# facebookresearch/moolib

Measured on AMD Instinct MI355X. Metric: env frames/sec (whole node) IMPALA Atari-ResNet, higher is better.
Workload: dtype bf16; 1 GPU; model=IMPALA Atari deep ResNet (16/32/32ch, FC3872-256), global_batch=32, seq_len=20, parallelism=dp1, actor_batch_size=128, num_actor_batches=2, num_actor_cpus=10, virtual_batch_size=32, num_actions=18, frame=84x84x4 uint8

## Files before the change

### hip/conv3x3.hip.inc

```

namespace conv3x3 {

using bf16 = __bf16;
using bf16x8 = __attribute__((ext_vector_type(8))) __bf16;
using floatx4 = __attribute__((ext_vector_type(4))) float;

#define C3_DEV static __device__ __forceinline__

C3_DEV bf16x8 zero8() {
  bf16x8 z;
#pragma unroll
  for (int e = 0; e < 8; ++e) z[e] = (bf16)0.f;
  return z;
}

enum { kEpiNone = 0, kEpiBias = 1, kEpiBiasRelu = 2, kEpiBiasAdd = 3 };

template <int C, bool RELU_IN, int RT>
__global__ __launch_bounds__(256) void conv3x3_nhwc_kernel(
    const bf16* __restrict__ x,
    const bf16* __restrict__ wPacked,
    const bf16* __restrict__ biasIn,
    bf16* __restrict__ out,
    const bf16* __restrict__ bias1,
    const bf16* __restrict__ res,
    const bf16* __restrict__ bias2,
    int NB, int H, int W, int K, int epi) {
  constexpr int KK = (9 * C + 31) / 32;
  const int lane = threadIdx.x & 63;
  const int wave = threadIdx.x >> 6;
  const int lo = lane & 15, hi = lane >> 4;
  const int64_t M = (int64_t)NB * H * W;
  const int64_t pixBase = ((int64_t)blockIdx.x * 4 + wave) * (16 * RT);
  if (pixBase >= M) return;

  int an[RT], aoh[RT], aow[RT];
  bool aok[RT];
#pragma unroll
  for (int rt = 0; rt < RT; ++rt) {
    const int64_t apix = pixBase + rt * 16 + lo;
    aok[rt] = apix < M;
    an[rt] = aoh[rt] = aow[rt] = 0;
    if (aok[rt]) {
      int64_t r = apix;
      aow[rt] = (int)(r % W);
      r /= W;
      aoh[rt] = (int)(r % H);
      an[rt] = (int)(r / H);
    }
  }
  const int nCt = K >> 4;
  constexpr int CH = (RT == 1) ? 2 : RT;
  floatx4 acc[CH][2];
#pragma unroll
  for (int ch = 0; ch < CH; ++ch)
#pragma unroll
    for (int ct = 0; ct < 2; ++ct) acc[ch][ct] = (floatx4){0.f, 0.f, 0.f, 0.f};

#pragma unroll
  for (int kk = 0; kk < KK; ++kk) {
    const int kd = kk * 32 + hi * 8;
    const int tap = kd / C;
    const int c0 = kd % C;
    bf16x8 a[RT];
#pragma unroll
    for (int rt = 0; rt < RT; ++rt) {
      a[rt] = zero8();
      if (aok[rt] && tap < 9) {
        const int ih = aoh[rt] + tap / 3 - 1;
        const int iw = aow[rt] + tap % 3 - 1;
        if (ih >= 0 && ih < H && iw >= 0 && iw < W) {
          const bf16* p = x + ((((int64_t)an[rt] * H + ih) * W + iw) * C + c0);
          a[rt] = *reinterpret_cast<const bf16x8*>(p);
          if (RELU_IN) {
#pragma unroll
            for (int e = 0; e < 8; ++e) {
              float v = (float)a[rt][e];
              if (biasIn != nullptr) v += (float)biasIn[c0 + e];
              a[rt][e] = (bf16)(v > 0.f ? v : 0.f);
            }
          }
        }
      }
    }
    for (int ct = 0; ct < nCt; ++ct) {
      const bf16* bp = wPacked + (((int64_t)ct * KK + kk) * 64 + lane) * 8;
      bf16x8 b = *reinterpret_cast<const bf16x8*>(bp);
#pragma unroll
      for (int rt = 0; rt < RT; ++rt) {
        const int ch = (RT == 1) ? (kk & 1) : rt;
        acc[ch][ct] = __builtin_amdgcn_mfma_f32_16x16x32_bf16(a[rt], b, acc[ch][ct], 0, 0, 0);
      }
    }
  }

#pragma unroll
  for (int rt = 0; rt < RT; ++rt) {
    for (int ct = 0; ct < nCt; ++ct) {
      const int col = ct * 16 + lo;
      const float b1 = (bias1 != nullptr) ? (float)bias1[col] : 0.f;
      const float b2 = (bias2 != nullptr) ? (float)bias2[col] : 0.f;
#pragma unroll
      for (int reg = 0; reg < 4; ++reg) {
        const int64_t pix = pixBase + rt * 16 + hi * 4 + reg;
        if (pix >= M) continue;
        float v = (RT == 1) ? (acc[0][ct][reg] + acc[1][ct][reg]) : acc[rt][ct][reg];
        if (epi == kEpiBias) {
          v += b1;
        } else if (epi == kEpiBiasRelu) {
          v += b1;
          v = v > 0.f ? v : 0.f;
        } else if (epi == kEpiBiasAdd) {
          v += b1 + b2 + (float)res[pix * K + col];
        }
        out[pix * K + col] = (bf16)v;
      }
    }
  }
}

template <int C, bool RELU_IN>
__global__ __launch_bounds__(256) void conv3x3_nhwc_lds_kernel(
    const bf16* __restrict__ x, const bf16* __restrict__ wPacked,
    const bf16* __restrict__ biasIn, bf16* __restrict__ out,
    const bf16* __restrict__ bias1, const bf16* __restrict__ res,
    const bf16* __restrict__ bias2, int NB, int H, int W, int K, int epi, int BR) {
  constexpr int KK = (9 * C + 31) / 32;
  const int lane = threadIdx.x & 63;
  const int wave = threadIdx.x >> 6;
  const int lo = lane & 15, hi = lane >> 4;
  const int nCt = K >> 4;
  const int WS = W + 2;

  extern __shared__ char smem[];
  bf16* slab = reinterpret_cast<bf16*>(smem);

  const int bandsPerImage = (H + BR - 1) / BR;
  const int band = blockIdx.x % bandsPerImage;
  const int n = blockIdx.x / bandsPerImage;
  const int row0 = band * BR;
  const int bandRows = min(BR, H - row0);
  const int bandPix = bandRows * W;

  constexpr int C8 = C / 8;
  {
    for (int idx = threadIdx.x; idx < (BR + 2) * WS * C8; idx += blockDim.x) {
      int c8 = idx % C8;
      int rest = idx / C8;
      int col = rest % WS;
      int sr = rest / WS;
      if (sr >= bandRows + 2) break;
      const int ih = row0 + sr - 1;
      const int iw = col - 1;
      bf16x8 v = zero8();
      if (ih >= 0 && ih < H && iw >= 0 && iw < W) {
        v = *reinterpret_cast<const bf16x8*>(
            x + ((((int64_t)n * H + ih) * W + iw) * C + c8 * 8));
        if (RELU_IN) {
#pragma unroll
          for (int e = 0; e < 8; ++e) {
            float f = (float)v[e];
            if (biasIn != nullptr) f += (float)biasIn[c8 * 8 + e];
            v[e] = (bf16)(f > 0.f ? f : 0.f);
          }
        }
      }
      *reinterpret_cast<bf16x8*>(slab + ((int64_t)sr * WS + col) * C + c8 * 8) = v;
    }
  }
  __syncthreads();

  const int nTiles = (bandPix + 15) / 16;
  for (int tile = wave; tile < nTiles; tile += 4) {
    const int p = tile * 16 + lo;
    const bool aok = p < bandPix;
    const int pr = aok ? p / W : 0;
    const int pc = aok ? p % W : 0;
    floatx4 acc[2][2];
#pragma unroll
    for (int pq = 0; pq < 2; ++pq)
#pragma unroll
      for (int ct = 0; ct < 2; ++ct) acc[pq][ct] = (floatx4){0.f, 0.f, 0.f, 0.f};
#pragma unroll
    for (int kk = 0; kk < KK; ++kk) {
      const int kd = kk * 32 + hi * 8;
      const int tap = kd / C;
      const int c0 = kd % C;
      bf16x8 a = zero8();
      if (aok && tap < 9) {
        const int sr = pr + tap / 3;
        const int sc = pc + tap % 3;
        a = *reinterpret_cast<const bf16x8*>(slab + ((int64_t)sr * WS + sc) * C + c0);
      }
      for (int ct = 0; ct < nCt; ++ct) {
        const bf16* bp = wPacked + (((int64_t)ct * KK + kk) * 64 + lane) * 8;
        bf16x8 b = *reinterpret_cast<const bf16x8*>(bp);
        acc[kk & 1][ct] = __builtin_amdgcn_mfma_f32_16x16x32_bf16(a, b, acc[kk & 1][ct], 0, 0, 0);
      }
    }
    const int64_t imgBase = ((int64_t)n * H + row0) * W;
    for (int ct = 0; ct < nCt; ++ct) {
      const int col = ct * 16 + lo;
      const float b1 = (bias1 != nullptr) ? (float)bias1[col] : 0.f;
      const float b2 = (bias2 != nullptr) ? (float)bias2[col] : 0.f;
#pragma unroll
      for (int reg = 0; reg < 4; ++reg) {
        const int pp = tile * 16 + hi * 4 + reg;
        if (pp >= bandPix) continue;
        const int64_t pix = imgBase + pp;
        float v = acc[0][ct][reg] + acc[1][ct][reg];
        if (epi == kEpiBias) {
          v += b1;
        } else if (epi == kEpiBiasRelu) {
          v += b1;
          v = v > 0.f ? v : 0.f;
        } else if (epi == kEpiBiasAdd) {
          v += b1 + b2 + (float)res[pix * K + col];
        }
        out[pix * K + col] = (bf16)v;
      }
    }
  }
}

}

at::Tensor conv3x3_nhwc_fused(at::Tensor x, at::Tensor wPacked, int64_t K,
                              bool reluIn, c10::optional<at::Tensor> biasIn,
                              int64_t epi, c10::optional<at::Tensor> bias1,
                              c10::optional<at::Tensor> res,
                              c10::optional<at::Tensor> bias2,
                              int64_t rtOverride) {
  TORCH_CHECK(x.is_cuda() && x.dim() == 4 && x.scalar_type() == at::kBFloat16,
              "conv3x3: bf16 4D CUDA tensor expected");
  TORCH_CHECK(x.is_contiguous(at::MemoryFormat::ChannelsLast), "conv3x3: channels_last expected");
  const int NB = x.size(0), C = x.size(1), H = x.size(2), W = x.size(3);
  TORCH_CHECK(C == 8 || C == 16 || C == 32, "conv3x3: C in {8,16,32}");
  TORCH_CHECK(K == 16 || K == 32, "conv3x3: K in {16,32}");
  TORCH_CHECK(epi >= conv3x3::kEpiNone && epi <= conv3x3::kEpiBiasAdd, "conv3x3: epi in 0..3");
  TORCH_CHECK(rtOverride <= 0 || rtOverride == 1 || rtOverride == 2 || rtOverride == 4,
              "conv3x3: rt in {1,2,4}");
  auto checkVec = [&](const at::Tensor& t, int64_t n, const char* name) {
    TORCH_CHECK(t.is_cuda() && t.device() == x.device() && t.scalar_type() == at::kBFloat16 &&
                    t.is_contiguous(),
                "conv3x3: ", name, " must be a contiguous bf16 tensor on x's device");
    TORCH_CHECK(t.numel() == n, "conv3x3: ", name, " has ", t.numel(), " elements, expected ", n);
  };
  checkVec(wPacked, (int64_t)((9 * C + 31) / 32) * 32 * K, "w_packed");
  if (biasIn.has_value()) checkVec(*biasIn, C, "bias_in");
  TORCH_CHECK(epi == conv3x3::kEpiNone || bias1.has_value(), "conv3x3: epi ", epi,
              " needs bias1");
  if (bias1.has_value()) checkVec(*bias1, K, "bias1");
  if (bias2.has_value()) checkVec(*bias2, K, "bias2");
  TORCH_CHECK(epi != conv3x3::kEpiBiasAdd || res.has_value(), "conv3x3: epi 3 needs res");
  if (res.has_value()) {
    TORCH_CHECK(res->is_cuda() && res->device() == x.device() &&
                    res->scalar_type() == at::kBFloat16,
                "conv3x3: res must be a bf16 tensor on x's device");
    TORCH_CHECK(res->dim() == 4 && res->size(0) == NB && res->size(1) == K &&
                    res->size(2) == H && res->size(3) == W,
                "conv3x3: res must have the output's shape [N,K,H,W]");
    TORCH_CHECK(res->is_contiguous(at::MemoryFormat::ChannelsLast),
                "conv3x3: res channels_last expected");
  }
  auto out = at::empty({NB, K, H, W},
                       x.options().memory_format(at::MemoryFormat::ChannelsLast));
  const int64_t M = (int64_t)NB * H * W;
  const int rt = rtOverride > 0 ? (int)rtOverride : (M >= 512 * 1024) ? 2 : 1;
  const int64_t blocks = (M + 64 * rt - 1) / (64 * rt);
  hipStream_t stream = c10::hip::getCurrentHIPStream().stream();
  using conv3x3::bf16;
  auto bf = [](const c10::optional<at::Tensor>& t) -> const bf16* {
    return t.has_value() ? reinterpret_cast<const bf16*>(t->data_ptr()) : nullptr;
  };
  const bf16* xp = reinterpret_cast<const bf16*>(x.data_ptr());
  const bf16* wp = reinterpret_cast<const bf16*>(wPacked.data_ptr());
  bf16* op = reinterpret_cast<bf16*>(out.data_ptr());

  static const bool ldsVariant = []() {
    const char* e = std::getenv("MOOLIB_AMD_CONV3_LDS");
    return e != nullptr && e[0] != '0';
  }();
  if (ldsVariant && rtOverride >= 0) {
    const int WS = W + 2;
    int BR = (int)(32768 / ((int64_t)WS * C * 2)) - 2;
    BR = std::min(BR, H);
    if (BR >= 4) {
      const size_t lds = (size_t)(BR + 2) * WS * C * 2;
      const int bandsPerImage = (H + BR - 1) / BR;
      const int64_t lblocks = (int64_t)NB * bandsPerImage;
#define C3_LDS_LAUNCH(CC, RIN)                                                       \
  hipLaunchKernelGGL((conv3x3::conv3x3_nhwc_lds_kernel<CC, RIN>), dim3(lblocks),     \
                     dim3(256), lds, stream, xp, wp, bf(biasIn), op, bf(bias1),      \
                     bf(res), bf(bias2), NB, H, W, (int)K, (int)epi, BR)
      if (C == 8) {
        if (reluIn) C3_LDS_LAUNCH(8, true); else C3_LDS_LAUNCH(8, false);
      } else if (C == 16) {
        if (reluIn) C3_LDS_LAUNCH(16, true); else C3_LDS_LAUNCH(16, false);
      } else {
        if (reluIn) C3_LDS_LAUNCH(32, true); else C3_LDS_LAUNCH(32, false);
      }
#undef C3_LDS_LAUNCH
      return out;
    }
  }
#define C3_LAUNCH(CC, RIN, RTT)                                                     \
  hipLaunchKernelGGL((conv3x3::conv3x3_nhwc_kernel<CC, RIN, RTT>), dim3(blocks),    \
                     dim3(256), 0, stream, xp, wp, bf(biasIn), op, bf(bias1),       \
                     bf(res), bf(bias2), NB, H, W, (int)K, (int)epi)
#define C3_RT(CC, RIN)                                                              \
  do {                                                                              \
    if (rt == 4) C3_LAUNCH(CC, RIN, 4);                                             \
    else if (rt == 2) C3_LAUNCH(CC, RIN, 2);                                        \
    else C3_LAUNCH(CC, RIN, 1);                                                     \
  } while (0)
  if (C == 8) {
    if (reluIn) C3_RT(8, true); else C3_RT(8, false);
  } else if (C == 16) {
    if (reluIn) C3_RT(16, true); else C3_RT(16, false);
  } else {
    if (reluIn) C3_RT(32, true); else C3_RT(32, false);
  }
#undef C3_RT
#undef C3_LAUNCH
  return out;
}
```

### hip/kernels.hip

```cpp
#include <hip/hip_runtime.h>
#include <hip/hip_bf16.h>
#include <torch/extension.h>
#include <c10/hip/HIPStream.h>

#include <climits>
#include <cstdlib>
#include <vector>

#define DEV_INLINE __device__ __forceinline__

namespace {

constexpr int kWave = 64;


__global__ void vtrace_scan_kernel(const float* __restrict__ log_rhos,
                                   const float* __restrict__ discounts,
                                   const float* __restrict__ rewards,
                                   const float* __restrict__ values,
                                   const float* __restrict__ bootstrap,
                                   float* __restrict__ vs,
                                   float* __restrict__ pg_advantages, int T, int B,
                                   float rho_bar, float pg_rho_bar) {
  int b = blockIdx.x * blockDim.x + threadIdx.x;
// ... 702 lines not shown
  checkNhwcPair(x, "channel_sum");
  int C = x.size(1);
  TORCH_CHECK(C <= 64, "channel_sum: C <= 64 (LDS accumulator)");
  auto out = at::zeros({C}, x.options().dtype(at::kFloat));
  int64_t total8 = x.numel() / 8;
  int threads = 256;
  int64_t blockCap = std::min<int64_t>(std::max<int64_t>(total8 / 3000, 256), 768);
  int64_t blocks = channelSumBlocks(total8, threads, blockCap, C / 8);
  hipStream_t stream = c10::hip::getCurrentHIPStream().stream();
  AT_DISPATCH_FLOATING_TYPES_AND2(
      at::kBFloat16, at::kHalf, x.scalar_type(), "channel_sum", [&] {
        hipLaunchKernelGGL(channel_sum_kernel<scalar_t>, dim3(blocks), dim3(threads), 0, stream,
                           x.data_ptr<scalar_t>(), out.data_ptr<float>(), total8, C / 8);
      });
  return out;
}

at::Tensor bias_add2_fwd(at::Tensor x, at::Tensor b1, at::Tensor s,
                         c10::optional<at::Tensor> b2) {
  checkNhwcPair(x, "bias_add2");
  checkNhwcPair(s, "bias_add2(shortcut)");
  int C = x.size(1);
  TORCH_CHECK(b1.numel() == C && b1.scalar_type() == x.scalar_type(), "bias_add2: bad bias1");
  at::Tensor b2c;
  if (b2.has_value()) {
    TORCH_CHECK(b2->numel() == C && b2->scalar_type() == x.scalar_type(), "bias_add2: bad bias2");
    b2c = b2->contiguous();
  }
  auto out = at::empty_like(x, x.options().memory_format(at::MemoryFormat::ChannelsLast));
  int64_t total8 = x.numel() / 8;
  int threads = 256;
  int64_t blocks = (total8 + threads - 1) / threads;
  hipStream_t stream = c10::hip::getCurrentHIPStream().stream();
  AT_DISPATCH_FLOATING_TYPES_AND2(
      at::kBFloat16, at::kHalf, x.scalar_type(), "bias_add2_fwd", [&] {
        hipLaunchKernelGGL(bias_add2_fwd_kernel<scalar_t>, dim3(blocks), dim3(threads), 0, stream,
                           x.data_ptr<scalar_t>(), b1.contiguous().data_ptr<scalar_t>(),
                           s.data_ptr<scalar_t>(),
                           b2.has_value() ? b2c.data_ptr<scalar_t>() : nullptr,
                           out.data_ptr<scalar_t>(), total8, C / 8);
      });
  return out;
}


struct CopyDesc {
  const uint8_t* src;
  uint8_t* dst;
  int64_t rows;
  int64_t rowBytes;
  int64_t srcStrideB;
  int64_t dstStrideB;
  int32_t vec;
  int32_t pad;
};

constexpr int kMaxCopyDescs = 24;
struct CopyDescPack {
  CopyDesc d[kMaxCopyDescs];
  int32_t n;
};

template <typename V>
DEV_INLINE void copyRun(const CopyDesc& e, int64_t start, int64_t step, int64_t total) {
  for (int64_t idx = start; idx < total; idx += step) {
    int64_t byte = idx * (int64_t)sizeof(V);
    int64_t row = byte / e.rowBytes;
    int64_t col = byte - row * e.rowBytes;
    *reinterpret_cast<V*>(e.dst + row * e.dstStrideB + col) =
        *reinterpret_cast<const V*>(e.src + row * e.srcStrideB + col);
  }
}

__global__ void batched_copy_kernel(CopyDescPack pack) {
  const CopyDesc& e = pack.d[blockIdx.y];
  int64_t units = e.rows * e.rowBytes / e.vec;
  int64_t start = (int64_t)blockIdx.x * blockDim.x + threadIdx.x;
  int64_t step = (int64_t)gridDim.x * blockDim.x;
  if (e.vec == 16) copyRun<uint4>(e, start, step, units);
  else if (e.vec == 4) copyRun<uint32_t>(e, start, step, units);
  else copyRun<uint8_t>(e, start, step, units);
}

namespace {

bool rowDecompose(const at::Tensor& t, int64_t& rows, int64_t& rowElems, int64_t& strideEl) {
  int64_t inner = 1;
  int d = t.dim() - 1;
  for (; d >= 0; --d) {
    if (t.size(d) == 1) continue;
    if (t.stride(d) != inner) break;
    inner *= t.size(d);
  }
  rowElems = inner;
  if (d < 0) {
    rows = 1;
    strideEl = inner;
    return true;
  }
  rows = t.size(d);
  strideEl = t.stride(d);
  for (int i = d - 1; i >= 0; --i) {
    if (t.size(i) == 1) continue;
    if (t.stride(i) != strideEl * rows) return false;
    rows *= t.size(i);
  }
  return strideEl >= rowElems;
}

int vecWidthFor(const void* a, const void* b, int64_t rowBytes, int64_t sA, int64_t sB) {
  auto ok = [&](int64_t v) {
    return ((uintptr_t)a % v == 0) && ((uintptr_t)b % v == 0) && (rowBytes % v == 0) &&
           (sA % v == 0) && (sB % v == 0);
  };
  if (ok(16)) return 16;
  if (ok(4)) return 4;
  return 1;
}

}

void batched_copy(std::vector<at::Tensor> dsts, std::vector<at::Tensor> srcs) {
  TORCH_CHECK(dsts.size() == srcs.size(), "batched_copy: length mismatch");
  CopyDescPack pack;
  pack.n = 0;
  int64_t maxUnits = 0;
  hipStream_t stream = c10::hip::getCurrentHIPStream().stream();
  auto flush = [&]() {
    if (pack.n == 0) return;
    int threads = 256;
    int64_t blocksX = std::min<int64_t>((maxUnits + threads - 1) / threads, 1024);
    hipLaunchKernelGGL(batched_copy_kernel, dim3(blocksX, pack.n), dim3(threads), 0, stream,
                       pack);
    pack.n = 0;
    maxUnits = 0;
  };
  for (size_t i = 0; i < dsts.size(); ++i) {
    at::Tensor& dst = dsts[i];
    at::Tensor& src = srcs[i];
    bool fused = false;
    if (dst.is_cuda() && src.is_cuda() && dst.device() == src.device() &&
        dst.scalar_type() == src.scalar_type() && dst.numel() == src.numel() &&
        dst.numel() > 0) {
      int64_t dRows, dRowEl, dStride, sRows, sRowEl, sStride;
      if (rowDecompose(dst, dRows, dRowEl, dStride) &&
          rowDecompose(src, sRows, sRowEl, sStride)) {
        if (dRows == 1 && sRows > 1) {
          dRows = sRows;
          dRowEl = sRowEl;
          dStride = sRowEl;
        } else if (sRows == 1 && dRows > 1) {
          sRows = dRows;
          sRowEl = dRowEl;
          sStride = dRowEl;
        }
        if (dRows == sRows && dRowEl == sRowEl) {
          int64_t esize = dst.element_size();
          CopyDesc e;
          e.src = (const uint8_t*)src.data_ptr();
          e.dst = (uint8_t*)dst.data_ptr();
          e.rows = dRows;
          e.rowBytes = dRowEl * esize;
          e.srcStrideB = sStride * esize;
          e.dstStrideB = dStride * esize;
          e.vec = vecWidthFor(e.src, e.dst, e.rowBytes, e.srcStrideB, e.dstStrideB);
          pack.d[pack.n++] = e;
          maxUnits = std::max(maxUnits, e.rows * e.rowBytes / e.vec);
          if (pack.n == kMaxCopyDescs) flush();
          fused = true;
        }
      }
    }
    if (!fused) dst.copy_(src, true);
  }
  flush();
}

#include "replay.hip.inc"

#include "act.hip.inc"

#include "optim.hip.inc"


namespace repack3x3 {

using bf16 = __bf16;

struct Desc {
  const bf16* w;
  bf16* outF;
  bf16* outD;
  int64_t sK, sC, sH, sW;
  int32_t C, K;
  int32_t Cp;
};
constexpr int kMaxDescs = 20;
struct Pack {
  Desc d[kMaxDescs];
  int32_t n;
};

__global__ void repack3x3_kernel(Pack pack) {
  const Desc& d = pack.d[blockIdx.y];
  const int KKf = (9 * d.Cp + 31) / 32;
  const int KKd = (9 * d.K + 31) / 32;
  const int nF = d.outF ? KKf * 32 * d.K : 0;
  const int nD = d.outD ? KKd * 32 * d.C : 0;
  for (int i = blockIdx.x * blockDim.x + threadIdx.x; i < nF + nD;
       i += gridDim.x * blockDim.x) {
    const bool isF = i < nF;
    const int idx = isF ? i : i - nF;
    const int KK = isF ? KKf : KKd;
    const int CC = isF ? d.Cp : d.K;
    const int e = idx & 7;
    const int lane = (idx >> 3) & 63;
    const int rest = idx >> 9;
    const int kk = rest % KK;
    const int ct = rest / KK;
    const int kd = kk * 32 + (lane >> 4) * 8 + e;
    const int n = ct * 16 + (lane & 15);
    bf16 v = (bf16)0.f;
    if (kd < 9 * CC) {
      const int tap = kd / CC, c = kd % CC;
      const int kh = tap / 3, kw = tap % 3;
      if (isF) {
        if (c < d.C) v = d.w[n * d.sK + c * d.sC + kh * d.sH + kw * d.sW];
      } else {
        v = d.w[c * d.sK + n * d.sC + (2 - kh) * d.sH + (2 - kw) * d.sW];
      }
    }
    (isF ? d.outF : d.outD)[idx] = v;
  }
}

}

void repack3x3_batched(std::vector<at::Tensor> ws, std::vector<at::Tensor> fwdBufs,
                       std::vector<at::Tensor> dgradBufs, std::vector<int64_t> packChannels) {
  TORCH_CHECK(ws.size() == fwdBufs.size() && ws.size() == dgradBufs.size() &&
                  ws.size() == packChannels.size(),
              "repack3x3: list length mismatch");
  hipStream_t stream = c10::hip::getCurrentHIPStream().stream();
  repack3x3::Pack pack;
  pack.n = 0;
  auto flush = [&]() {
    if (pack.n == 0) return;
    hipLaunchKernelGGL(repack3x3::repack3x3_kernel, dim3(32, pack.n), dim3(256), 0, stream,
                       pack);
    pack.n = 0;
  };
  for (size_t i = 0; i < ws.size(); ++i) {
    at::Tensor& w = ws[i];
    TORCH_CHECK(w.is_cuda() && w.dim() == 4 && w.scalar_type() == at::kBFloat16,
                "repack3x3: bf16 4D CUDA weight expected");
    const int K = w.size(0), C = w.size(1);
    repack3x3::Desc e;
    e.w = reinterpret_cast<const repack3x3::bf16*>(w.data_ptr());
    e.sK = w.stride(0);
    e.sC = w.stride(1);
    e.sH = w.stride(2);
    e.sW = w.stride(3);
    e.C = C;
    e.K = K;
    e.Cp = packChannels[i] > C ? (int)packChannels[i] : C;
    e.outF = nullptr;
    e.outD = nullptr;
    if (fwdBufs[i].defined() && fwdBufs[i].numel() > 0) {
      TORCH_CHECK(fwdBufs[i].numel() == (9 * e.Cp + 31) / 32 * 32 * K, "repack3x3: fwd size");
      e.outF = reinterpret_cast<repack3x3::bf16*>(fwdBufs[i].data_ptr());
    }
    if (dgradBufs[i].defined() && dgradBufs[i].numel() > 0) {
      TORCH_CHECK(dgradBufs[i].numel() == (9 * K + 31) / 32 * 32 * C, "repack3x3: dgrad size");
      e.outD = reinterpret_cast<repack3x3::bf16*>(dgradBufs[i].data_ptr());
    }
    pack.d[pack.n++] = e;
    if (pack.n == repack3x3::kMaxDescs) flush();
  }
  flush();
}

PYBIND11_MODULE(TORCH_EXTENSION_NAME, m) {
  m.doc() = "moolib_amd gfx950 HIP kernels";
  m.def("register_host_memory", &register_host_memory);
  m.def("repack3x3_batched", &repack3x3_batched,
        "refresh all conv MFMA weight packs (fwd + dgrad) in one launch");
  m.def("batched_copy", &batched_copy,
        "copy many (dst<-src) slice pairs in one kernel launch (gfx950)");
  m.def("maxpool3x3s2_fwd", &maxpool3x3s2_fwd, "NHWC 3x3/2 maxpool forward (gfx950)");
  m.def("maxpool3x3s2_bwd", &maxpool3x3s2_bwd, "NHWC 3x3/2 maxpool backward (gather, no atomics)");
  m.def("bias_relu_fwd", &bias_relu_fwd, "fused conv-bias + relu, one NHWC pass (gfx950)");
  m.def("bias_relu_bwd", &bias_relu_bwd, "bias_relu backward: dx + fp32 db in one pass");
  m.def("bias_add2_fwd", &bias_add2_fwd, "fused residual close: x + bias1 + shortcut (+ bias2)");
  m.def("channel_sum_fp32", &channel_sum_fp32,
        "NHWC per-channel fp32 sum (bias gradients; small-grid atomics)");
  m.def("frames_u8_to_bf16_nhwc", &frames_u8_to_bf16_nhwc,
        "fused uint8->bf16 NHWC scale (optionally zero-padding channels)",
        py::arg("x"), py::arg("scale"), py::arg("pad_channels") = 0);
  m.def("conv1_u8_nhwc", &conv1_u8_nhwc, "fused uint8 frames -> conv(4->16,3x3)+bias, NHWC bf16");
  m.def("conv3x3_nhwc_fused", &conv3x3_nhwc_fused,
        "MFMA 3x3/s1/p1 NHWC conv with fused relu/bias prologue + bias/relu/residual epilogue",
        py::arg("x"), py::arg("w_packed"), py::arg("k"), py::arg("relu_in") = false,
        py::arg("bias_in") = py::none(), py::arg("epi") = 0, py::arg("bias1") = py::none(),
        py::arg("res") = py::none(), py::arg("bias2") = py::none(), py::arg("rt") = 0);
  m.def("wgrad3x3_nhwc", &wgrad3x3_nhwc,
        "3x3/s1/p1 conv weight gradient on MFMA (row-slab LDS staging, gfx950)");
  m.def("lstm_fused_fwd", &lstm_fused_fwd, "fused masked LSTM sequence scan fwd (MFMA, gfx950)");
  m.def("lstm_fused_bwd", &lstm_fused_bwd, "fused masked LSTM sequence scan bwd (MFMA, gfx950)");
  m.def("vtrace_from_log_rhos", &vtrace_from_log_rhos, "fused V-trace scan (gfx950)");
  m.def("impala_loss", &impala_loss, "fused IMPALA loss fwd+grad (gfx950)");
  m.def("r2d2_loss", &r2d2_loss,
        "fused R2D2 loss: n-step double-Q TD errors, sequence loss, priorities, grad_q (gfx950)",
        py::arg("q"), py::arg("q_target"), py::arg("actions"), py::arg("rewards"),
        py::arg("discounts"), py::arg("mask"), py::arg("is_weights"), py::arg("n"),
        py::arg("eps"), py::arg("rescale"), py::arg("eta"), py::arg("grad_scale"),
        py::arg("grad_out") = py::none());
  m.def("r2d2_actor_priority", &r2d2_actor_priority,
        "initial sequence priorities [K] and TD errors [T,K] from an actor's q_taken / q_max, "
        "reward and done in the actor's layout; one launch (gfx950)",
        py::arg("q_taken"), py::arg("q_max"), py::arg("reward"), py::arg("done"), py::arg("n"),
        py::arg("discount"), py::arg("eps"), py::arg("rescale"), py::arg("eta"),
        py::arg("burn_in"), py::arg("priority_out") = py::none(),
        py::arg("td_out") = py::none());
  m.attr("R2D2_MAX_T") = r2d2::kMaxT;
  m.def("replay_tree_update", &replay_tree_update,
        "sum-tree leaves <- priority^alpha (last wins), ancestors, max_priority (gfx950)",
        py::arg("tree"), py::arg("max_priority"), py::arg("slots"), py::arg("priorities"),
        py::arg("alpha"), py::arg("L"));
  m.def("replay_tree_sample", &replay_tree_sample,
        "stratified sum-tree sample: idx [B], normalised importance weights [B] (gfx950)",
        py::arg("tree"), py::arg("L"), py::arg("size"), py::arg("u"), py::arg("beta"),
        py::arg("idx_out") = py::none(), py::arg("weights_out") = py::none());
  m.def("replay_rows", &replay_rows,
        "gather / scatter whole items of every nest leaf by a device index, one launch",
        py::arg("storage"), py::arg("other"), py::arg("index"), py::arg("mode"));
  m.attr("REPLAY_MAX_UPDATE") = replay::kMaxUpdate;
  m.attr("REPLAY_MAX_SAMPLE") = replay::kMaxSample;
  m.def("act_categorical", &act_categorical,
        "action ~ softmax(logits) from [seed, step] Philox state or explicit uniforms (gfx950)",
        py::arg("logits"), py::arg("state") = py::none(), py::arg("u") = py::none(),
        py::arg("action_out") = py::none());
  m.def("act_eps_greedy", &act_eps_greedy,
        "epsilon-greedy dueling head: action, q_taken, q_max in one launch (gfx950)",
        py::arg("value"), py::arg("advantage"), py::arg("epsilon"), py::arg("state") = py::none(),
        py::arg("u") = py::none(), py::arg("action_out") = py::none(),
        py::arg("q_taken_out") = py::none(), py::arg("q_max_out") = py::none());
  m.attr("ACT_MAX_ACTIONS") = act::kMaxActions;
  m.def("flat_adam_step", &flat_adam_step,
        "fused flat Adam: grad norm, clip, update of p/m/v, bf16 shadow; two launches (gfx950)",
        py::arg("p"), py::arg("g"), py::arg("m"), py::arg("v"), py::arg("shadow"),
        py::arg("step"), py::arg("step_next"), py::arg("lr"), py::arg("partial"),
        py::arg("norm_out"), py::arg("beta1"), py::arg("beta2"), py::arg("eps"),
        py::arg("max_norm") = py::none());
  m.attr("FLAT_ADAM_MAX_BLOCKS") = optim::kMaxBlocks;
  m.attr("FLAT_ADAM_PASS_ELEMENTS") = optim::kPassElements;
}
```

### moolib_amd/ops/conv3x3.py

```python
import os

import torch
import torch.nn.functional as F
from torch import nn

from moolib_amd.ops.lstm import pack_mfma_b

EPI_NONE, EPI_BIAS, EPI_BIAS_RELU, EPI_BIAS_ADD = 0, 1, 2, 3

_kernels = None


def _k():
    global _kernels
    if _kernels is None:
        from moolib_amd import _kernels as k

        _kernels = k
    return _kernels


def kernels():
    try:
        return _k()
    except ImportError:
        return None


def available(C, K):
    if os.environ.get("MOOLIB_AMD_CONV3_KERNEL", "1") == "0":
        return False
    if C not in (16, 32) or K not in (16, 32):
        return False
    return kernels() is not None


def bf16_compute(t):
    return t.dtype == torch.bfloat16 or torch.is_autocast_enabled()


def runs_on_mfma(x, C, K):
    return x.is_cuda and available(C, K) and bf16_compute(x)


def pack_weight(w):
    K, C, kh, kw = w.shape
    assert kh == 3 and kw == 3
    gem = w.permute(2, 3, 1, 0).reshape(9 * C, K)
    kk32 = (9 * C + 31) // 32 * 32
    if kk32 != 9 * C:
        gem = torch.cat([gem, gem.new_zeros(kk32 - 9 * C, K)])
    return pack_mfma_b(gem.to(torch.bfloat16).contiguous())


def pack_weight_dgrad(w):
    wd = w.flip(2, 3).permute(1, 0, 2, 3).contiguous()
    return pack_weight(wd)


def pack_weight_c8(w):
    return pack_weight(F.pad(w, (0, 0, 0, 0, 0, 8 - w.shape[1])))


PACKERS = {"fwd": pack_weight, "dgrad": pack_weight_dgrad, "c8": pack_weight_c8}


def _refresh(entry, kind, w):
    entry[1].copy_(PACKERS[kind](w.detach()))
    entry[0] = w._version


def packed(conv, kind="fwd"):
    w = conv.weight
    packs = conv.__dict__.setdefault("_c3_packs", {})
    entry = packs.get(kind)
    if entry is None:
        packs[kind] = entry = [w._version, PACKERS[kind](w.detach())]
    elif entry[0] != w._version:
        _refresh(entry, kind, w)
    return entry[1]


def repack(module):
    ws, fs, ds, cps, batched = [], [], [], [], []
    for m in module.modules():
        packs = getattr(m, "_c3_packs", None) if isinstance(m, nn.Conv2d) else None
        if not packs:
            continue
        w = m.weight.detach()
        if not (w.is_cuda and w.dtype == torch.bfloat16):
            for kind, entry in packs.items():
                _refresh(entry, kind, m.weight)
            continue
        fwd, dgrad, c8 = (packs.get(kind) for kind in ("fwd", "dgrad", "c8"))
        if fwd is not None or dgrad is not None:
            ws.append(w)
            fs.append(fwd[1] if fwd is not None else w.new_empty(0))
            ds.append(dgrad[1] if dgrad is not None else w.new_empty(0))
            cps.append(0)
        if c8 is not None:
            ws.append(w)
            fs.append(c8[1])
            ds.append(w.new_empty(0))
            cps.append(8)
        batched.append(m)
    if ws:
        _k().repack3x3_batched(ws, fs, ds, cps)
        for m in batched:
            for entry in m._c3_packs.values():
                entry[0] = m.weight._version


class _Conv3x3Fn(torch.autograd.Function):

    @staticmethod
    def forward(ctx, x, weight, conv_module):
        xb = x.to(torch.bfloat16).contiguous(memory_format=torch.channels_last)
        y = conv3x3(xb, packed(conv_module), weight.shape[0])
        ctx.save_for_backward(xb, weight)
        ctx.conv_module = conv_module
        ctx.x_dtype = x.dtype
        return y

    @staticmethod
    def backward(ctx, dy):
        x, w = ctx.saved_tensors
        m = ctx.conv_module
        dy = dy.to(torch.bfloat16).contiguous(memory_format=torch.channels_last)
        dx = dw = None
        if ctx.needs_input_grad[0]:
            dx = conv3x3(dy, packed(m, "dgrad"), w.shape[1])
            if dx.dtype != ctx.x_dtype:
                dx = dx.to(ctx.x_dtype)
        if ctx.needs_input_grad[1]:
            if os.environ.get("MOOLIB_AMD_WGRAD_KERNEL"):
                K, C = w.shape[0], w.shape[1]
                g = _k().wgrad3x3_nhwc(x, dy)[: 9 * C]
                dw = g.view(3, 3, C, K).permute(3, 2, 0, 1)
            else:
                wb = w if w.dtype == dy.dtype else w.to(dy.dtype)
                dw = torch.ops.aten.convolution_backward(
                    dy, x, wb, None, [1, 1], [1, 1], [1, 1], False, [0, 0], 1,
                    [False, True, False],
                )[1]
            if dw.dtype != w.dtype:
                dw = dw.to(w.dtype)
        return dx, dw, None


def conv3x3_autograd(x, conv_module):
    return _Conv3x3Fn.apply(x, conv_module.weight, conv_module)


def _conv1_u8(x_u8, conv, scale):
    xb8 = _k().frames_u8_to_bf16_nhwc(x_u8, scale, 8)
    y = conv3x3(
        xb8, packed(conv, "c8"), conv.out_channels,
        epi=EPI_BIAS, bias1=conv.bias.detach(),
    )
    return xb8, y


class _Conv1U8Fn(torch.autograd.Function):

    @staticmethod
    def forward(ctx, x_u8, weight, bias, conv_module, scale):
        xb8, y = _conv1_u8(x_u8, conv_module, scale)
        ctx.save_for_backward(xb8, weight)
        return y

    @staticmethod
    def backward(ctx, dy):
        xb8, w = ctx.saved_tensors
        k = _k()
        dyb = dy.to(torch.bfloat16).contiguous(memory_format=torch.channels_last)
        K, C = w.shape[0], w.shape[1]
        g = k.wgrad3x3_nhwc(xb8, dyb)[: 9 * 8]
        dw = g.view(3, 3, 8, K)[:, :, :C].permute(3, 2, 0, 1).to(w.dtype)
        db = k.channel_sum_fp32(dyb).to(w.dtype)
        return None, dw, db, None, None


def conv1_u8_autograd(x_u8, conv_module, scale):
    if torch.is_grad_enabled() and conv_module.weight.requires_grad:
        return _Conv1U8Fn.apply(
            x_u8, conv_module.weight, conv_module.bias, conv_module, scale
        )
    return _conv1_u8(x_u8, conv_module, scale)[1]


def conv3x3(x, w_packed, k, relu_in=False, bias_in=None, epi=EPI_NONE,
            bias1=None, res=None, bias2=None, rt=0):
    to_bf = lambda t: None if t is None else t.to(torch.bfloat16)
    return _k().conv3x3_nhwc_fused(
        x.to(torch.bfloat16).contiguous(memory_format=torch.channels_last),
        w_packed,
        k,
        relu_in,
        to_bf(bias_in),
        epi,
        to_bf(bias1),
        None if res is None else to_bf(res).contiguous(memory_format=torch.channels_last),
        to_bf(bias2),
        rt,
    )
```

Measured before the change: 86680 frames/s.

## Rewrite flat conv3x3 kernel as persistent grid with LDS-staged weights and vectorized epilogue

The flat NHWC 3x3 conv kernel now stages all packed weights in LDS once per block and runs a persistent grid sized from CU count and occupancy, with each wave looping over 16-pixel tiles. Per-lane tap offsets and a validity bitmask are precomputed, 64-bit div/mod is replaced by magic-number fast division, and all input taps are loaded up front. The epilogue swaps the MFMA operand order so each lane holds four contiguous channels, giving vectorized bf16x4 stores and residual loads, with biases hoisted out of the loop. K is now a template parameter. This aims to cut repeated global weight loads, index arithmetic, and scattered scalar stores, at the cost of an LDS fill per block, more template instantiations, and a host-side occupancy query.

Result: faster. 95220 frames/s, median of 5 (+9.8%).

```diff
diff --git a/hip/conv3x3.hip.inc b/hip/conv3x3.hip.inc
--- a/hip/conv3x3.hip.inc
+++ b/hip/conv3x3.hip.inc
@@ -3,6 +3,7 @@
 
 using bf16 = __bf16;
 using bf16x8 = __attribute__((ext_vector_type(8))) __bf16;
+using bf16x4 = __attribute__((ext_vector_type(4))) __bf16;
 using floatx4 = __attribute__((ext_vector_type(4))) float;
 
 #define C3_DEV static __device__ __forceinline__
@@ -16,7 +17,171 @@
 
 enum { kEpiNone = 0, kEpiBias = 1, kEpiBiasRelu = 2, kEpiBiasAdd = 3 };
 
-template <int C, bool RELU_IN, int RT>
+constexpr int kkChunks(int C) { return (9 * C + 31) / 32; }
+
+template <int KK>
+struct MemWeights {
+  const bf16x8* base;
+  __device__ __forceinline__ MemWeights(const bf16x8* frags, int lane) : base(frags + lane) {}
+  __device__ __forceinline__ bf16x8 operator()(int kk, int ct) const {
+    return base[(ct * KK + kk) * 64];
+  }
+};
+
+template <int NCT>
+struct EpiBias {
+  float b1[NCT][4], b2[NCT][4];
+  __device__ __forceinline__ EpiBias(const bf16* bias1, const bf16* bias2, int hi) {
+#pragma unroll
+    for (int ct = 0; ct < NCT; ++ct)
+#pragma unroll
+      for (int r = 0; r < 4; ++r) {
+        const int ch = ct * 16 + 4 * hi + r;
+        b1[ct][r] = (bias1 != nullptr) ? (float)bias1[ch] : 0.f;
+        b2[ct][r] = (bias2 != nullptr) ? (float)bias2[ch] : 0.f;
+      }
+  }
+};
+
+C3_DEV bf16x8 reluIn(bf16x8 a, const float (&bin)[8]) {
+#pragma unroll
+  for (int e = 0; e < 8; ++e) {
+    const float v = (float)a[e] + bin[e];
+    a[e] = (bf16)(v > 0.f ? v : 0.f);
+  }
+  return a;
+}
+
+template <int KK, int NCT, bool DUAL, class WF>
+C3_DEV void accumulateTile(const bf16x8 (&a)[KK], const WF& wf, floatx4 (&acc)[NCT]) {
+  constexpr int CH = DUAL ? 2 : 1;
+  floatx4 chain[CH][NCT];
+#pragma unroll
+  for (int ch = 0; ch < CH; ++ch)
+#pragma unroll
+    for (int ct = 0; ct < NCT; ++ct) chain[ch][ct] = (floatx4){0.f, 0.f, 0.f, 0.f};
+#pragma unroll
+  for (int kk = 0; kk < KK; ++kk) {
+    const int ch = DUAL ? (kk & 1) : 0;
+#pragma unroll
+    for (int ct = 0; ct < NCT; ++ct)
+      chain[ch][ct] =
+          __builtin_amdgcn_mfma_f32_16x16x32_bf16(wf(kk, ct), a[kk], chain[ch][ct], 0, 0, 0);
+  }
+#pragma unroll
+  for (int ct = 0; ct < NCT; ++ct) {
+    if (DUAL) {
+#pragma unroll
+      for (int r = 0; r < 4; ++r) acc[ct][r] = chain[0][ct][r] + chain[CH - 1][ct][r];
+    } else {
+      acc[ct] = chain[0][ct];
+    }
+  }
+}
+
+template <int NCT>
+C3_DEV void epilogueStore(const floatx4 (&acc)[NCT], int epi, const EpiBias<NCT>& eb,
+                          const bf16x4 (&resv)[NCT], bf16* outp) {
+#pragma unroll
+  for (int ct = 0; ct < NCT; ++ct) {
+    bf16x4 o;
+#pragma unroll
+    for (int r = 0; r < 4; ++r) {
+      float v = acc[ct][r];
+      if (epi == kEpiBias) {
+        v += eb.b1[ct][r];
+      } else if (epi == kEpiBiasRelu) {
+        v += eb.b1[ct][r];
+        v = v > 0.f ? v : 0.f;
+      } else if (epi == kEpiBiasAdd) {
+        v += eb.b1[ct][r] + eb.b2[ct][r] + (float)resv[ct][r];
+      }
+      o[r] = (bf16)v;
+    }
+    *reinterpret_cast<bf16x4*>(outp + ct * 16) = o;
+  }
+}
+
+struct FastDiv {
+  uint32_t m, sh;
+  FastDiv() = default;
+  explicit FastDiv(uint32_t d) {
+    uint32_t l = 0;
+    while ((1ull << l) < d) ++l;
+    sh = 31 + l;
+    m = (uint32_t)(((1ull << sh) + d - 1) / d);
+  }
+  __device__ __forceinline__ uint32_t operator()(uint32_t n) const {
+    return (uint32_t)(((uint64_t)n * m) >> sh);
+  }
+};
+
+template <int C>
+struct LaneTaps {
+  static constexpr int KK = kkChunks(C);
+  static constexpr int LPT = C / 8;
+  static constexpr int TPK = 32 / C;
+  int off[KK];
+  int hiTap;
+  int c0;
+  __device__ __forceinline__ LaneTaps(int hi, int W) {
+    hiTap = hi / LPT;
+    c0 = (hi % LPT) * 8;
+#pragma unroll
+    for (int kk = 0; kk < KK; ++kk) {
+      const int tap = kk * TPK + hiTap;
+      const int dh = tap / 3 - 1, dw = tap % 3 - 1;
+      off[kk] = tap < 9 ? ((dh * W + dw) * C + c0) * 2 : 0;
+    }
+  }
+};
+
+template <int KK, int NCT>
+struct TileIn {
+  bf16x8 a[KK];
+  bf16x4 r[NCT];
+  unsigned valid;
+  unsigned pix;
+};
+
+template <int C, int K>
+C3_DEV void loadTile(TileIn<kkChunks(C), K / 16>& t, int tile,
+                     const LaneTaps<C>& lt, const char* __restrict__ xb,
+                     const char* __restrict__ resb, int M, int H, int W, FastDiv divW,
+                     FastDiv divH, int epi, int lo, int hi) {
+  constexpr int KK = kkChunks(C);
+  constexpr int NCT = K / 16;
+  constexpr int TPK = 32 / C;
+  const int p = tile * 16 + lo;
+  const bool ok = p < M;
+  const unsigned pc = ok ? (unsigned)p : 0u;
+  const unsigned row = divW(pc);
+  const int ow = (int)(pc - row * (unsigned)W);
+  const int oh = (int)(row - divH(row) * (unsigned)H);
+  const unsigned cols = ((ow > 0 ? 1u : 0u) | 2u | (ow < W - 1 ? 4u : 0u)) * 0x49u;
+  const unsigned rows = (oh > 0 ? 0x7u : 0u) | 0x38u | (oh < H - 1 ? 0x1c0u : 0u);
+  const unsigned laneValid = ok ? ((cols & rows) >> lt.hiTap) : 0u;
+  const unsigned pixByte = pc * (unsigned)(C * 2);
+  t.pix = pc;
+  t.valid = laneValid | (ok ? 0x80000000u : 0u);
+#pragma unroll
+  for (int kk = 0; kk < KK; ++kk) {
+    const unsigned o = (laneValid >> (kk * TPK)) & 1u ? pixByte + (unsigned)lt.off[kk] : 0u;
+    t.a[kk] = *reinterpret_cast<const bf16x8*>(xb + o);
+  }
+  if (epi == kEpiBiasAdd) {
+#pragma unroll
+    for (int ct = 0; ct < NCT; ++ct)
+      t.r[ct] = *reinterpret_cast<const bf16x4*>(resb + (pc * (unsigned)(K * 2) + ct * 32 + 8 * hi));
+  } else {
+#pragma unroll
+    for (int ct = 0; ct < NCT; ++ct)
+#pragma unroll
+      for (int r = 0; r < 4; ++r) t.r[ct][r] = (bf16)0.f;
+  }
+}
+
+template <int C, int K, bool RELU_IN, bool DUAL>
 __global__ __launch_bounds__(256) void conv3x3_nhwc_kernel(
     const bf16* __restrict__ x,
     const bf16* __restrict__ wPacked,
@@ -25,111 +190,65 @@
     const bf16* __restrict__ bias1,
     const bf16* __restrict__ res,
     const bf16* __restrict__ bias2,
-    int NB, int H, int W, int K, int epi) {
-  constexpr int KK = (9 * C + 31) / 32;
+    int M, int H, int W, FastDiv divW, FastDiv divH, int epi, int nTiles, int tilesPerBlock) {
+  constexpr int KK = kkChunks(C);
+  constexpr int NCT = K / 16;
+  constexpr int TPK = 32 / C;
   const int lane = threadIdx.x & 63;
   const int wave = threadIdx.x >> 6;
   const int lo = lane & 15, hi = lane >> 4;
-  const int64_t M = (int64_t)NB * H * W;
-  const int64_t pixBase = ((int64_t)blockIdx.x * 4 + wave) * (16 * RT);
-  if (pixBase >= M) return;
-
-  int an[RT], aoh[RT], aow[RT];
-  bool aok[RT];
-#pragma unroll
-  for (int rt = 0; rt < RT; ++rt) {
-    const int64_t apix = pixBase + rt * 16 + lo;
-    aok[rt] = apix < M;
-    an[rt] = aoh[rt] = aow[rt] = 0;
-    if (aok[rt]) {
-      int64_t r = apix;
-      aow[rt] = (int)(r % W);
-      r /= W;
-      aoh[rt] = (int)(r % H);
-      an[rt] = (int)(r / H);
-    }
-  }
-  const int nCt = K >> 4;
-  constexpr int CH = (RT == 1) ? 2 : RT;
-  floatx4 acc[CH][2];
-#pragma unroll
-  for (int ch = 0; ch < CH; ++ch)
-#pragma unroll
-    for (int ct = 0; ct < 2; ++ct) acc[ch][ct] = (floatx4){0.f, 0.f, 0.f, 0.f};
-
-#pragma unroll
-  for (int kk = 0; kk < KK; ++kk) {
-    const int kd = kk * 32 + hi * 8;
-    const int tap = kd / C;
-    const int c0 = kd % C;
-    bf16x8 a[RT];
-#pragma unroll
-    for (int rt = 0; rt < RT; ++rt) {
-      a[rt] = zero8();
-      if (aok[rt] && tap < 9) {
-        const int ih = aoh[rt] + tap / 3 - 1;
-        const int iw = aow[rt] + tap % 3 - 1;
-        if (ih >= 0 && ih < H && iw >= 0 && iw < W) {
-          const bf16* p = x + ((((int64_t)an[rt] * H + ih) * W + iw) * C + c0);
-          a[rt] = *reinterpret_cast<const bf16x8*>(p);
-          if (RELU_IN) {
-#pragma unroll
-            for (int e = 0; e < 8; ++e) {
-              float v = (float)a[rt][e];
-              if (biasIn != nullptr) v += (float)biasIn[c0 + e];
-              a[rt][e] = (bf16)(v > 0.f ? v : 0.f);
-            }
-          }
-        }
-      }
-    }
-    for (int ct = 0; ct < nCt; ++ct) {
-      const bf16* bp = wPacked + (((int64_t)ct * KK + kk) * 64 + lane) * 8;
-      bf16x8 b = *reinterpret_cast<const bf16x8*>(bp);
-#pragma unroll
-      for (int rt = 0; rt < RT; ++rt) {
-        const int ch = (RT == 1) ? (kk & 1) : rt;
-        acc[ch][ct] = __builtin_amdgcn_mfma_f32_16x16x32_bf16(a[rt], b, acc[ch][ct], 0, 0, 0);
-      }
-    }
-  }
-
-#pragma unroll
-  for (int rt = 0; rt < RT; ++rt) {
-    for (int ct = 0; ct < nCt; ++ct) {
-      const int col = ct * 16 + lo;
-      const float b1 = (bias1 != nullptr) ? (float)bias1[col] : 0.f;
-      const float b2 = (bias2 != nullptr) ? (float)bias2[col] : 0.f;
-#pragma unroll
-      for (int reg = 0; reg < 4; ++reg) {
-        const int64_t pix = pixBase + rt * 16 + hi * 4 + reg;
-        if (pix >= M) continue;
-        float v = (RT == 1) ? (acc[0][ct][reg] + acc[1][ct][reg]) : acc[rt][ct][reg];
-        if (epi == kEpiBias) {
-          v += b1;
-        } else if (epi == kEpiBiasRelu) {
-          v += b1;
-          v = v > 0.f ? v : 0.f;
-        } else if (epi == kEpiBiasAdd) {
-          v += b1 + b2 + (float)res[pix * K + col];
-        }
-        out[pix * K + col] = (bf16)v;
-      }
-    }
-  }
-}
-
-template <int C, bool RELU_IN>
+
+  __shared__ bf16x8 wsh[KK * NCT * 64];
+  for (int i = threadIdx.x; i < KK * NCT * 64; i += 256)
+    wsh[i] = reinterpret_cast<const bf16x8*>(wPacked)[i];
+  __syncthreads();
+
+  const int first = blockIdx.x * tilesPerBlock + wave;
+  const int tileEnd = min((int)(blockIdx.x + 1) * tilesPerBlock, nTiles);
+  if (first >= tileEnd) return;
+
+  const MemWeights<KK> wf(wsh, lane);
+  const EpiBias<NCT> eb(bias1, bias2, hi);
+  const LaneTaps<C> lt(hi, W);
+  const bool hasBin = RELU_IN && biasIn != nullptr;
+  float bin[8];
+#pragma unroll
+  for (int e = 0; e < 8; ++e) bin[e] = hasBin ? (float)biasIn[lt.c0 + e] : 0.f;
+  const char* xb = reinterpret_cast<const char*>(x);
+  const char* resb = reinterpret_cast<const char*>(res);
+  char* outb = reinterpret_cast<char*>(out);
+
+  for (int tile = first; tile < tileEnd; tile += 4) {
+    TileIn<KK, NCT> cur;
+    loadTile<C, K>(cur, tile, lt, xb, resb, M, H, W, divW, divH, epi, lo, hi);
+    asm volatile("" ::: "memory");
+
+    bf16x8 a[KK];
+#pragma unroll
+    for (int kk = 0; kk < KK; ++kk) {
+      bf16x8 v = cur.a[kk];
+      if (RELU_IN) v = reluIn(v, bin);
+      a[kk] = ((cur.valid >> (kk * TPK)) & 1u) ? v : zero8();
+    }
+    floatx4 acc[NCT];
+    accumulateTile<KK, NCT, DUAL>(a, wf, acc);
+    if (cur.valid >> 31)
+      epilogueStore<NCT>(acc, epi, eb, cur.r,
+                         reinterpret_cast<bf16*>(outb + (cur.pix * (unsigned)(K * 2) + 8 * hi)));
+  }
+}
+
+template <int C, int K, bool RELU_IN>
 __global__ __launch_bounds__(256) void conv3x3_nhwc_lds_kernel(
     const bf16* __restrict__ x, const bf16* __restrict__ wPacked,
     const bf16* __restrict__ biasIn, bf16* __restrict__ out,
     const bf16* __restrict__ bias1, const bf16* __restrict__ res,
-    const bf16* __restrict__ bias2, int NB, int H, int W, int K, int epi, int BR) {
-  constexpr int KK = (9 * C + 31) / 32;
+    const bf16* __restrict__ bias2, int NB, int H, int W, int epi, int BR) {
+  constexpr int KK = kkChunks(C);
+  constexpr int NCT = K / 16;
   const int lane = threadIdx.x & 63;
   const int wave = threadIdx.x >> 6;
   const int lo = lane & 15, hi = lane >> 4;
-  const int nCt = K >> 4;
   const int WS = W + 2;
 
   extern __shared__ char smem[];
@@ -170,56 +289,106 @@
   }
   __syncthreads();
 
+  const MemWeights<KK> wf(reinterpret_cast<const bf16x8*>(wPacked), lane);
+  const EpiBias<NCT> eb(bias1, bias2, hi);
+  const int64_t imgBase = ((int64_t)n * H + row0) * W;
+
   const int nTiles = (bandPix + 15) / 16;
   for (int tile = wave; tile < nTiles; tile += 4) {
     const int p = tile * 16 + lo;
     const bool aok = p < bandPix;
     const int pr = aok ? p / W : 0;
     const int pc = aok ? p % W : 0;
-    floatx4 acc[2][2];
-#pragma unroll
-    for (int pq = 0; pq < 2; ++pq)
-#pragma unroll
-      for (int ct = 0; ct < 2; ++ct) acc[pq][ct] = (floatx4){0.f, 0.f, 0.f, 0.f};
+    bf16x8 a[KK];
 #pragma unroll
     for (int kk = 0; kk < KK; ++kk) {
       const int kd = kk * 32 + hi * 8;
       const int tap = kd / C;
       const int c0 = kd % C;
-      bf16x8 a = zero8();
+      a[kk] = zero8();
       if (aok && tap < 9) {
         const int sr = pr + tap / 3;
         const int sc = pc + tap % 3;
-        a = *reinterpret_cast<const bf16x8*>(slab + ((int64_t)sr * WS + sc) * C + c0);
-      }
-      for (int ct = 0; ct < nCt; ++ct) {
-        const bf16* bp = wPacked + (((int64_t)ct * KK + kk) * 64 + lane) * 8;
-        bf16x8 b = *reinterpret_cast<const bf16x8*>(bp);
-        acc[kk & 1][ct] = __builtin_amdgcn_mfma_f32_16x16x32_bf16(a, b, acc[kk & 1][ct], 0, 0, 0);
-      }
-    }
-    const int64_t imgBase = ((int64_t)n * H + row0) * W;
-    for (int ct = 0; ct < nCt; ++ct) {
-      const int col = ct * 16 + lo;
-      const float b1 = (bias1 != nullptr) ? (float)bias1[col] : 0.f;
-      const float b2 = (bias2 != nullptr) ? (float)bias2[col] : 0.f;
-#pragma unroll
-      for (int reg = 0; reg < 4; ++reg) {
-        const int pp = tile * 16 + hi * 4 + reg;
-        if (pp >= bandPix) continue;
-        const int64_t pix = imgBase + pp;
-        float v = acc[0][ct][reg] + acc[1][ct][reg];
-        if (epi == kEpiBias) {
-          v += b1;
-        } else if (epi == kEpiBiasRelu) {
-          v += b1;
-          v = v > 0.f ? v : 0.f;
-        } else if (epi == kEpiBiasAdd) {
-          v += b1 + b2 + (float)res[pix * K + col];
+        a[kk] = *reinterpret_cast<const bf16x8*>(slab + ((int64_t)sr * WS + sc) * C + c0);
+      }
+    }
+    floatx4 acc[NCT];
+    accumulateTile<KK, NCT, true>(a, wf, acc);
+    if (aok) {
+      const int64_t pix = imgBase + p;
+      bf16x4 resv[NCT];
+#pragma unroll
+      for (int ct = 0; ct < NCT; ++ct) {
+        if (epi == kEpiBiasAdd) {
+          resv[ct] = *reinterpret_cast<const bf16x4*>(res + (pix * K + ct * 16 + 4 * hi));
+        } else {
+#pragma unroll
+          for (int r = 0; r < 4; ++r) resv[ct][r] = (bf16)0.f;
         }
-        out[pix * K + col] = (bf16)v;
-      }
-    }
+      }
+      epilogueStore<NCT>(acc, epi, eb, resv, out + (pix * K + 4 * hi));
+    }
+  }
+}
+
+inline bool notCapturing(hipStream_t stream) {
+  hipStreamCaptureStatus cs = hipStreamCaptureStatusNone;
+  return hipStreamIsCapturing(stream, &cs) == hipSuccess && cs == hipStreamCaptureStatusNone;
+}
+
+inline int cuCount(int dev, hipStream_t stream) {
+  static int cached[64] = {0};
+  if (dev < 0 || dev >= 64) return 256;
+  if (cached[dev] == 0) {
+    if (!notCapturing(stream)) return 256;
+    int n = 0;
+    if (hipDeviceGetAttribute(&n, hipDeviceAttributeMultiprocessorCount, dev) != hipSuccess ||
+        n <= 0)
+      n = 256;
+    cached[dev] = n;
+  }
+  return cached[dev];
+}
+
+struct FlatArgs {
+  const bf16 *x, *w, *biasIn, *bias1, *res, *bias2;
+  bf16* out;
+  int M, H, W, epi, dev;
+  int64_t maxBlocks;
+  hipStream_t stream;
+};
+
+template <int C, int K, bool RIN, bool DUAL>
+void launchFlat(const FlatArgs& a) {
+  auto kernel = conv3x3_nhwc_kernel<C, K, RIN, DUAL>;
+  static int perCu = 0;
+  int resident = perCu;
+  if (resident == 0) {
+    resident = 2;
+    if (notCapturing(a.stream)) {
+      int n = 0;
+      if (hipOccupancyMaxActiveBlocksPerMultiprocessor(&n, kernel, 256, 0) == hipSuccess && n > 0)
+        resident = n;
+      perCu = resident;
+    }
+  }
+  const int nTiles = (a.M + 15) / 16;
+  int64_t cap = (int64_t)cuCount(a.dev, a.stream) * resident;
+  if (a.maxBlocks > 0) cap = std::min<int64_t>(cap, a.maxBlocks);
+  int blocks = (int)std::min<int64_t>(cap, (nTiles + 3) / 4);
+  const int tilesPerBlock = (nTiles + blocks - 1) / blocks;
+  blocks = (nTiles + tilesPerBlock - 1) / tilesPerBlock;
+  hipLaunchKernelGGL(kernel, dim3(blocks), dim3(256), 0, a.stream, a.x, a.w, a.biasIn, a.out,
+                     a.bias1, a.res, a.bias2, a.M, a.H, a.W, FastDiv((uint32_t)a.W),
+                     FastDiv((uint32_t)a.H), a.epi, nTiles, tilesPerBlock);
+}
+
+template <int C, int K>
+void launchFlatCK(const FlatArgs& a, bool reluIn, bool dual) {
+  if (reluIn) {
+    if (dual) launchFlat<C, K, true, true>(a); else launchFlat<C, K, true, false>(a);
+  } else {
+    if (dual) launchFlat<C, K, false, true>(a); else launchFlat<C, K, false, false>(a);
   }
 }
 
@@ -230,7 +399,7 @@
                               int64_t epi, c10::optional<at::Tensor> bias1,
                               c10::optional<at::Tensor> res,
                               c10::optional<at::Tensor> bias2,
-                              int64_t rtOverride) {
+                              int64_t rtOverride, int64_t maxBlocks) {
   TORCH_CHECK(x.is_cuda() && x.dim() == 4 && x.scalar_type() == at::kBFloat16,
               "conv3x3: bf16 4D CUDA tensor expected");
   TORCH_CHECK(x.is_contiguous(at::MemoryFormat::ChannelsLast), "conv3x3: channels_last expected");
@@ -266,8 +435,12 @@
   auto out = at::empty({NB, K, H, W},
                        x.options().memory_format(at::MemoryFormat::ChannelsLast));
   const int64_t M = (int64_t)NB * H * W;
+  TORCH_CHECK(M <= (int64_t)INT_MAX - 64, "conv3x3: N*H*W = ", M, " must fit in int32");
+  TORCH_CHECK(M * std::max<int64_t>(C, K) * 2 <= (int64_t)UINT_MAX,
+              "conv3x3: input and output must be below 4 GiB each");
+  if (M == 0) return out;
   const int rt = rtOverride > 0 ? (int)rtOverride : (M >= 512 * 1024) ? 2 : 1;
-  const int64_t blocks = (M + 64 * rt - 1) / (64 * rt);
+  const bool dual = rt == 1;
   hipStream_t stream = c10::hip::getCurrentHIPStream().stream();
   using conv3x3::bf16;
   auto bf = [](const c10::optional<at::Tensor>& t) -> const bf16* {
@@ -289,39 +462,38 @@
       const size_t lds = (size_t)(BR + 2) * WS * C * 2;
       const int bandsPerImage = (H + BR - 1) / BR;
       const int64_t lblocks = (int64_t)NB * bandsPerImage;
-#define C3_LDS_LAUNCH(CC, RIN)                                                       \
-  hipLaunchKernelGGL((conv3x3::conv3x3_nhwc_lds_kernel<CC, RIN>), dim3(lblocks),     \
-                     dim3(256), lds, stream, xp, wp, bf(biasIn), op, bf(bias1),      \
-                     bf(res), bf(bias2), NB, H, W, (int)K, (int)epi, BR)
+#define C3_LDS_LAUNCH(CC, KK_, RIN)                                                    \
+  hipLaunchKernelGGL((conv3x3::conv3x3_nhwc_lds_kernel<CC, KK_, RIN>), dim3(lblocks),  \
+                     dim3(256), lds, stream, xp, wp, bf(biasIn), op, bf(bias1),        \
+                     bf(res), bf(bias2), NB, H, W, (int)epi, BR)
+#define C3_LDS_K(CC, RIN)                                                              \
+  do {                                                                                 \
+    if (K == 16) C3_LDS_LAUNCH(CC, 16, RIN); else C3_LDS_LAUNCH(CC, 32, RIN);          \
+  } while (0)
       if (C == 8) {
-        if (reluIn) C3_LDS_LAUNCH(8, true); else C3_LDS_LAUNCH(8, false);
+        if (reluIn) C3_LDS_K(8, true); else C3_LDS_K(8, false);
       } else if (C == 16) {
-        if (reluIn) C3_LDS_LAUNCH(16, true); else C3_LDS_LAUNCH(16, false);
+        if (reluIn) C3_LDS_K(16, true); else C3_LDS_K(16, false);
       } else {
-        if (reluIn) C3_LDS_LAUNCH(32, true); else C3_LDS_LAUNCH(32, false);
-      }
+        if (reluIn) C3_LDS_K(32, true); else C3_LDS_K(32, false);
+      }
+#undef C3_LDS_K
 #undef C3_LDS_LAUNCH
       return out;
     }
   }
-#define C3_LAUNCH(CC, RIN, RTT)                                                     \
-  hipLaunchKernelGGL((conv3x3::conv3x3_nhwc_kernel<CC, RIN, RTT>), dim3(blocks),    \
-                     dim3(256), 0, stream, xp, wp, bf(biasIn), op, bf(bias1),       \
-                     bf(res), bf(bias2), NB, H, W, (int)K, (int)epi)
-#define C3_RT(CC, RIN)                                                              \
-  do {                                                                              \
-    if (rt == 4) C3_LAUNCH(CC, RIN, 4);                                             \
-    else if (rt == 2) C3_LAUNCH(CC, RIN, 2);                                        \
-    else C3_LAUNCH(CC, RIN, 1);                                                     \
-  } while (0)
+
+  const conv3x3::FlatArgs fa{xp, wp, bf(biasIn), bf(bias1), bf(res), bf(bias2), op,
+                             (int)M, H, W, (int)epi, (int)x.get_device(), maxBlocks, stream};
   if (C == 8) {
-    if (reluIn) C3_RT(8, true); else C3_RT(8, false);
+    if (K == 16) conv3x3::launchFlatCK<8, 16>(fa, reluIn, dual);
+    else conv3x3::launchFlatCK<8, 32>(fa, reluIn, dual);
   } else if (C == 16) {
-    if (reluIn) C3_RT(16, true); else C3_RT(16, false);
+    if (K == 16) conv3x3::launchFlatCK<16, 16>(fa, reluIn, dual);
+    else conv3x3::launchFlatCK<16, 32>(fa, reluIn, dual);
   } else {
-    if (reluIn) C3_RT(32, true); else C3_RT(32, false);
-  }
-#undef C3_RT
-#undef C3_LAUNCH
+    if (K == 16) conv3x3::launchFlatCK<32, 16>(fa, reluIn, dual);
+    else conv3x3::launchFlatCK<32, 32>(fa, reluIn, dual);
+  }
   return out;
 }
diff --git a/hip/kernels.hip b/hip/kernels.hip
--- a/hip/kernels.hip
+++ b/hip/kernels.hip
@@ -1028,7 +1028,7 @@
         "MFMA 3x3/s1/p1 NHWC conv with fused relu/bias prologue + bias/relu/residual epilogue",
         py::arg("x"), py::arg("w_packed"), py::arg("k"), py::arg("relu_in") = false,
         py::arg("bias_in") = py::none(), py::arg("epi") = 0, py::arg("bias1") = py::none(),
-        py::arg("res") = py::none(), py::arg("bias2") = py::none(), py::arg("rt") = 0);
+        py::arg("res") = py::none(), py::arg("bias2") = py::none(), py::arg("rt") = 0, py::arg("max_blocks") = 0);
   m.def("wgrad3x3_nhwc", &wgrad3x3_nhwc,
         "3x3/s1/p1 conv weight gradient on MFMA (row-slab LDS staging, gfx950)");
   m.def("lstm_fused_fwd", &lstm_fused_fwd, "fused masked LSTM sequence scan fwd (MFMA, gfx950)");
diff --git a/moolib_amd/ops/conv3x3.py b/moolib_amd/ops/conv3x3.py
--- a/moolib_amd/ops/conv3x3.py
+++ b/moolib_amd/ops/conv3x3.py
@@ -190,7 +190,7 @@
 
 
 def conv3x3(x, w_packed, k, relu_in=False, bias_in=None, epi=EPI_NONE,
-            bias1=None, res=None, bias2=None, rt=0):
+            bias1=None, res=None, bias2=None, rt=0, max_blocks=0):
     to_bf = lambda t: None if t is None else t.to(torch.bfloat16)
     return _k().conv3x3_nhwc_fused(
         x.to(torch.bfloat16).contiguous(memory_format=torch.channels_last),
@@ -203,4 +203,5 @@
         None if res is None else to_bf(res).contiguous(memory_format=torch.channels_last),
         to_bf(bias2),
         rt,
+        max_blocks,
     )
```
